# rogosprojects/klogs

Measured on AMD Instinct MI355X. Metric: filtered log GB/s (whole node) at 1/2/4/8 MI355X; % of HBM peak, higher is better.
Workload: dtype u8

## Files before the change

### klogs_amd/csrc/klf_kernels.hip

```cpp
#include <hip/hip_ext.h>
#include <hip/hip_runtime.h>

#include <cstdio>
#include <cstdlib>
#include <cstring>
#include <type_traits>

#include "klf_kernels.hpp"
#include "klf_ts.hpp"

namespace klf {
namespace {

#ifndef KLF_TIMELINE
#define KLF_TIMELINE 0
#endif
__device__ uint32_t g_abl_waves;
#if KLF_TIMELINE
__device__ uint64_t g_timeline[300000 * 8];
__device__ uint32_t g_lb_rounds, g_lb_spins;
#define KLF_STAMP(tile, k) do { if (threadIdx.x == 0 && (tile) < 300000) g_timeline[(size_t)(tile) * 8 + (k)] = __builtin_amdgcn_s_memtime(); } while (0)
#else
#define KLF_STAMP(tile, k) do { } while (0)
#endif
// ... 163 lines not shown
    y.sel = (fl & 2) != 0;
    if (lane >= d) x = f_combine(y, x);
  }
  return x;
}

__device__ __forceinline__ uint32_t xad(uint32_t x, uint32_t c, uint32_t d) {
  uint32_t r;
  asm("v_xad_u32 %0, %1, %2, %3" : "=v"(r) : "v"(x), "s"(c), "v"(d));
  return r;
}
__device__ __forceinline__ uint32_t any_eq16(const uint4& v, uint32_t c4) {
  const uint32_t m = 0xFEFEFEFFu;
  return (xad(v.x, c4, m) | xad(v.y, c4, m) | xad(v.z, c4, m) | xad(v.w, c4, m)) & 0x80808080u;
}
__device__ __forceinline__ uint32_t eq_mask16(const uint4& v, uint32_t c4) {
  auto z = [c4](uint32_t x) {
    const uint32_t y = x ^ c4;
    const uint32_t f = ~(((y & 0x7F7F7F7Fu) + 0x7F7F7F7Fu) | y) & 0x80808080u;
    return (f * 0x00204081u) >> 28;
  };
  return z(v.x) | (z(v.y) << 4) | (z(v.z) << 8) | (z(v.w) << 12);
}

__device__ __forceinline__ uint32_t nor_and(uint32_t a, uint32_t b, uint32_t c) {
  uint32_t r;
  asm("v_bitop3_b32 %0, %1, %2, %3 bitop3:0x02" : "=v"(r) : "v"(a), "v"(b), "s"(c));
  return r;
}
__device__ __forceinline__ uint32_t eq_mask16_nl(const uint4& v) {
  auto z = [](uint32_t x) {
    const uint32_t t = xad(x & 0x7F7F7F7Fu, 0x0A0A0A0Au, 0x7F7F7F7Fu);
    const uint32_t f = nor_and(t, x, 0x80808080u);
    return (f * 0x00204081u) >> 28;
  };
  return z(v.x) | (z(v.y) << 4) | (z(v.z) << 8) | (z(v.w) << 12);
}

template <class T>
__device__ __forceinline__ T wave_max(T x) {
#pragma unroll
  for (int d = 32; d >= 1; d >>= 1) {
    const T o = __shfl_xor(x, d, 64);
    x = o > x ? o : x;
  }
  return x;
}

__device__ __forceinline__ void wave_lds_sync() { asm volatile("s_waitcnt lgkmcnt(0)" ::: "memory"); }

__global__ __launch_bounds__(256) void k_tiles(const SegDesc* segs, uint32_t nsegs, uint32_t ntiles,
                                               uint32_t* tile_seg) {
  for (uint32_t tile = blockIdx.x * 256 + threadIdx.x; tile < ntiles; tile += gridDim.x * 256)
    tile_seg[tile] = find_seg_by_tile(segs, nsegs, tile);
}

__device__ __forceinline__ uint32_t mul_hi_u24(uint32_t a, uint32_t b) {
  uint32_t r;
  asm("v_mul_hi_u32_u24 %0, %1, %2" : "=v"(r) : "s"(b), "v"(a));
  return r;
}
__device__ __forceinline__ uint32_t mul_u24(uint32_t a, uint32_t b) {
  uint32_t r;
  asm("v_mul_u32_u24 %0, %1, %2" : "=v"(r) : "s"(b), "v"(a));
  return r;
}
__device__ __forceinline__ uint32_t mad_u24(uint32_t a, uint32_t b, uint32_t c) {
  uint32_t r;
  asm("v_mad_u32_u24 %0, %1, %2, %3" : "=v"(r) : "v"(a), "s"(b), "v"(c));
  return r;
}
__device__ __forceinline__ uint32_t bfe_u32(uint32_t a, uint32_t off, uint32_t width) {
  uint32_t r;
  asm("v_bfe_u32 %0, %1, %2, %3" : "=v"(r) : "v"(a), "n"(off), "n"(width));
  return r;
}
__device__ __forceinline__ uint32_t shr_byte1(uint32_t w, uint32_t h) {
  uint32_t r;
  asm("v_lshrrev_b32_sdwa %0, %1, %2 dst_sel:DWORD dst_unused:UNUSED_PAD src0_sel:BYTE_1 src1_sel:DWORD"
      : "=v"(r) : "v"(h), "v"(w));
  return r;
}
#ifndef KLF_PARSE_UNALIGNED
#define KLF_PARSE_UNALIGNED 1
#endif
__device__ __forceinline__ bool parse_fast(const uint8_t* lds, uint32_t o, const uint32_t (&cut)[6], bool& since_ok) {
  uint32_t w[8];
  if (KLF_PARSE_UNALIGNED) {
    typedef uint32_t u32x4 __attribute__((ext_vector_type(4)));
    u32x4 x0, x1;
    __builtin_memcpy(&x0, lds + o, 16);
    __builtin_memcpy(&x1, lds + o + 16, 16);
    w[0] = x0.x; w[1] = x0.y; w[2] = x0.z; w[3] = x0.w;
    w[4] = x1.x; w[5] = x1.y; w[6] = x1.z; w[7] = x1.w;
  } else {
    const uint32_t* s32 = reinterpret_cast<const uint32_t*>(lds);
    const uint32_t base = o >> 2, sh = o & 3u;
    uint32_t prev = s32[base];
#pragma unroll
    for (int j = 0; j < 8; ++j) {
      const uint32_t nx = s32[base + j + 1];
      w[j] = __builtin_amdgcn_alignbyte(nx, prev, sh);
      prev = nx;
    }
  }
  const uint32_t sep = ((w[1] ^ 0x2D00002Du) & 0xFF0000FFu) | ((w[2] ^ 0x00540000u) & 0x00FF0000u) |
                       ((w[3] ^ 0x00003A00u) & 0x0000FF00u) | ((w[4] ^ 0x2E00003Au) & 0xFF0000FFu) |
                       ((w[7] ^ 0x00205A00u) & 0x00FFFF00u);
  const uint32_t p0 = __builtin_amdgcn_perm(0u, w[0], 0x00010203u);
  const uint32_t p1 = __builtin_amdgcn_perm(w[2], w[1], 0x01020405u);
  const uint32_t p2 = __builtin_amdgcn_perm(w[3], w[2], 0x03040607u);
  const uint32_t p3 = __builtin_amdgcn_perm(w[5], w[4], 0x01020405u);
  const uint32_t p4 = __builtin_amdgcn_perm(w[6], w[5], 0x02030405u);
  const uint32_t p5 = __builtin_amdgcn_perm(w[7], w[6], 0x02030C04u) | 0x00003000u;
  const uint32_t hi = ((p0 ^ 0x30303030u) | (p1 ^ 0x30303030u) | (p2 ^ 0x30303030u) | (p3 ^ 0x30303030u) |
                       (p4 ^ 0x30303030u) | (p5 ^ 0x30303030u)) & 0xF0F0F0F0u;
  const uint32_t lo = ((p0 + 0x06060606u) | (p1 + 0x06060606u) | (p2 + 0x06060606u) | (p3 + 0x06060606u) |
                       (p4 + 0x06060606u) | (p5 + 0x06060606u)) & 0x40404040u;
  if ((sep | hi | lo) != 0u) return false;
  if (p0 - 0x31393730u > 0x32303939u - 0x31393730u) return false;
  if ((p1 >> 16) - 0x3031u > 0x3132u - 0x3031u) return false;
  if ((p2 >> 16) > 0x3233u || (p2 & 0xFFFFu) > 0x3539u || (p3 >> 16) > 0x3539u) return false;
  if ((p1 & 0xFFFFu) - 0x3031u > 0x3238u - 0x3031u) {
    const uint32_t day = ((p1 >> 8) & 15u) * 10u + (p1 & 15u);
    const uint32_t month = ((p1 >> 24) & 15u) * 10u + ((p1 >> 16) & 15u);
    const uint32_t yy = ((p0 >> 8) & 15u) * 10u + (p0 & 15u);
    const uint32_t dim = month == 2u ? 28u + ((yy & 3u) == 0u ? 1u : 0u) : 30u + ((month + (month >> 3)) & 1u);
    if (day - 1u >= dim) return false;
  }
  const uint64_t a0 = (uint64_t)p0 << 32 | p1, a1 = (uint64_t)p2 << 32 | p3, a2 = (uint64_t)p4 << 32 | p5;
  const uint64_t c0 = (uint64_t)cut[0] << 32 | cut[1], c1 = (uint64_t)cut[2] << 32 | cut[3],
                 c2 = (uint64_t)cut[4] << 32 | cut[5];
  since_ok = a0 > c0 || (a0 == c0 && (a1 > c1 || (a1 == c1 && a2 >= c2)));
  return true;
}

#ifndef KLF_ABL
#define KLF_ABL 0
#endif
#ifndef KLF_SCAN_NT
#define KLF_SCAN_NT 1
#endif
#ifndef KLF_SCAN_PRIO
#define KLF_SCAN_PRIO 0
#endif
#ifndef KLF_NL_MASK
#define KLF_NL_MASK 1
#endif
#ifndef KLF_SCAN_BALLOT
#define KLF_SCAN_BALLOT 1
#endif
#ifndef KLF_SCAN_PACKSUM
#define KLF_SCAN_PACKSUM 1
#endif
#ifndef KLF_VERIFY_PAR
#define KLF_VERIFY_PAR 0
#endif
#ifndef KLF_HIT_INLINE
#define KLF_HIT_INLINE 0
#endif
#ifndef KLF_TS_INLINE
#define KLF_TS_INLINE 1
#endif
#ifndef KLF_SCAN_SUMSKIP
#define KLF_SCAN_SUMSKIP 1
#endif
typedef uint32_t klf_v4u __attribute__((ext_vector_type(4)));
__device__ __forceinline__ uint4 ld_nt(const uint4* p) {
  const klf_v4u v = __builtin_nontemporal_load(reinterpret_cast<const klf_v4u*>(p));
  return make_uint4(v.x, v.y, v.z, v.w);
}
#ifndef KLF_CG_NT
#define KLF_CG_NT 0
#endif
#ifndef KLF_CG_GRID
#define KLF_CG_GRID 8
#endif
#ifndef KLF_CG_PF2
#define KLF_CG_PF2 1
#endif
#ifndef KLF_COPY_U
#define KLF_COPY_U 1
#endif
#ifndef KLF_ANY_BATCH
#define KLF_ANY_BATCH 8
#endif
#ifndef KLF_SCAN_OCC
#define KLF_SCAN_OCC 3
#endif
constexpr int kScanPlain = 0, kScanLit = 1, kScanGen = 2;

__device__ __forceinline__ void copy_tile_runs(const uint8_t* s_buf, uint32_t* s_run, uint16_t* s_map, uint32_t nr,
                                               uint32_t kept, uint64_t obase, uint8_t* out, int lane);

template <int MODE, int QS, int QK, int QQ = 4, bool QA = false, bool FUSE = false>
__global__ __launch_bounds__(kThreads, MODE == kScanGen ? 3 : KLF_SCAN_OCC) void k_scan(RunArgs a, const uint32_t* __restrict__ tseg,
                                                               const SegDesc* __restrict__ segs) {
  static_assert(!FUSE || MODE == kScanPlain, "the fused compaction runs in the plain scan");
  constexpr bool LIT = MODE == kScanLit;
  constexpr bool GEN = MODE == kScanGen;
  constexpr bool ANC = GEN && QA;
  static_assert(QQ == 3 || QQ == 4, "3- or 4-byte grams");
  constexpr int kWaves = kThreads / 64;
  constexpr int kRows = kTile / 1024;
  constexpr int kPad = FUSE ? 16 : 0;
  __shared__ __attribute__((aligned(16))) uint8_t s_tile_all[kWaves][kPad + kTile + kHalo];
  __shared__ __attribute__((aligned(16))) uint32_t s_frun_all[FUSE ? kWaves : 1][FUSE ? kTcRuns : 1];
  __shared__ __attribute__((aligned(16))) uint16_t s_fmap_all[FUSE ? kWaves : 1][FUSE ? kTcChunks : 8];
  __shared__ __attribute__((aligned(16))) uint32_t s_list_all[kWaves][kSlotStride];
  __shared__ __attribute__((aligned(16))) uint32_t s_lit[kMaxFusedLiteral / 4 + 1];
  __shared__ uint4 s_gstat[GEN ? 1 : kWaves][kScanGroup];
  __shared__ uint32_t s_qf[GEN ? kQfWords : 1];
  __shared__ uint32_t s_h2[GEN ? kWaves : 1][1];
  const int t = threadIdx.x, lane = t & 63, wv = __builtin_amdgcn_readfirstlane(t >> 6);
  uint8_t* s_tile = s_tile_all[wv] + kPad;
  uint32_t* s_list = s_list_all[wv];
  uint32_t* err_flag = a.counters + 2;
  for (uint32_t i = t; i < kMaxFusedLiteral / 4 + 1; i += kThreads)
    s_lit[i] = (LIT && i < (a.lit_len + 3) / 4) ? a.lit_words[i] : 0u;
  if (GEN)
    for (uint32_t i = t; i < kQfWords; i += kThreads) s_qf[i] = a.pats.qf_bitmap[i];
  __syncthreads();
  const uint32_t nwaves = gridDim.x * kWaves;
  const bool abl = (KLF_ABL != 0) &&
                   __hip_atomic_load(&g_abl_waves, __ATOMIC_RELAXED, __HIP_MEMORY_SCOPE_AGENT) >= nwaves;
#define ABL(x) ((KLF_ABL & (x)) && abl)

  static_assert(kRows == 8, "KLF_ROWS lists the 8 prefetch rows");
#define KLF_ROWS(X) X(0) X(1) X(2) X(3) X(4) X(5) X(6) X(7)
#define KLF_DECL(r) uint4 pf##r;
  KLF_ROWS(KLF_DECL)
#undef KLF_DECL
#define KLF_LOAD(r) pf##r = (KLF_SCAN_NT && MODE != kScanPlain) ? ld_nt(&gp[r * 64 + lane]) : gp[r * 64 + lane];
#define KLF_STORE(r) l[r * 64 + lane] = pf##r;
  uint4 pfh = make_uint4(0, 0, 0, 0);
  auto next_tile = [&](uint32_t x) -> uint32_t {
    return (FUSE || (x % kScanGroup) != kScanGroup - 1) ? x + 1 : x + 1 + kScanGroup * (nwaves - 1);
  };
  const uint32_t gw = blockIdx.x * kWaves + wv;
  uint32_t tile = FUSE ? gw * a.fuse_range : gw * kScanGroup;
  const uint32_t tile_end = FUSE ? (tile + a.fuse_range < a.ntiles ? tile + a.fuse_range : a.ntiles) : a.ntiles;
  const uint32_t range_t0 = tile;
  uint4 stv = make_uint4(0, 0, 0, 0);
  uint32_t pf_s = 0;
  SegDesc pf_sd{};
  if (tile < a.ntiles) {
    pf_s = tseg[tile];
    pf_sd = segs[pf_s];
    const uint4* gp = reinterpret_cast<const uint4*>(a.bytes + pf_sd.base + (uint64_t)(tile - pf_sd.tile0) * kTile);
    KLF_ROWS(KLF_LOAD)
    if (lane < kHalo / 16) pfh = (KLF_SCAN_NT && MODE != kScanPlain) ? ld_nt(&gp[kTile / 16 + lane]) : gp[kTile / 16 + lane];
  }
  {
    const __amdgpu_buffer_rsrc_t none = __builtin_amdgcn_make_buffer_rsrc(a.slots, 0, 0, 0x00020000);
    __builtin_amdgcn_raw_buffer_store_b32(0u, none, 0x7FFF0000u, 0, 0);
  }
  bool any_defer = false;
  uint32_t wp_cur = 0, wp_end = 0;
  bool fz_known = false, fz_sel = false, fz_res_set = false;
  int32_t fz_crel = -1;
  uint64_t fz_obase = 0, fz_estart = 0, fz_res = 0, fz_part = 0, fz_rbase = 0;
  uint32_t fz_ext = 0;
  if (FUSE && tile < tile_end) {
    fz_rbase = pf_sd.base + (uint64_t)(tile - pf_sd.tile0) * kTile;
    fz_ext = a.fuse_ext0[gw];
  }
  auto fz_close = [&]() __attribute__((always_inline)) {
    if (!fz_res_set) {
      fz_res = fz_part;
      fz_res_set = true;
      fz_estart = fz_obase = fz_rbase + fz_part;
    }
    if (lane == 0) {
      a.fuse_ext[2 * (size_t)fz_ext] = fz_estart;
      a.fuse_ext[2 * (size_t)fz_ext + 1] = fz_obase - fz_estart;
    }
  };
  for (; tile < tile_end; tile = next_tile(tile)) {
    const uint32_t s = pf_s;
    const SegDesc sd = pf_sd;
    const int64_t rel_lo = (int64_t)(tile - sd.tile0) * kTile;
    const int64_t seg_len = (int64_t)sd.len;
    const int32_t tile_len = (int32_t)(seg_len - rel_lo < kTile ? seg_len - rel_lo : kTile);
    const bool first = rel_lo == 0;
    const bool last = rel_lo + kTile >= seg_len;
    const uint8_t* segp = a.bytes + sd.base;

    if (KLF_SCAN_PRIO) __builtin_amdgcn_s_setprio(KLF_SCAN_PRIO);
    {
      uint4* l = reinterpret_cast<uint4*>(s_tile);
      KLF_ROWS(KLF_STORE)
      if (lane < kHalo / 16) l[kTile / 16 + lane] = pfh;
      const uint32_t nx = next_tile(tile);
      if (nx < tile_end) {
        if (nx - sd.tile0 >= sd.ntiles) {
          pf_s = tseg[nx];
          pf_sd = segs[pf_s];
        }
        const uint4* gp = reinterpret_cast<const uint4*>(a.bytes + pf_sd.base + (uint64_t)(nx - pf_sd.tile0) * kTile);
        KLF_ROWS(KLF_LOAD)
        if (lane < kHalo / 16) pfh = (KLF_SCAN_NT && MODE != kScanPlain) ? ld_nt(&gp[kTile / 16 + lane]) : gp[kTile / 16 + lane];
      }
    }
    if (KLF_SCAN_PRIO) __builtin_amdgcn_s_setprio(0);
    wave_lds_sync();

    const uint32_t my0 = (uint32_t)lane * kLaneBytes;
    const int nvalid_s = tile_len - (int)my0;
    const int nvalid = nvalid_s <= 0 ? 0 : (nvalid_s >= kLaneBytes ? kLaneBytes : nvalid_s);
// ... 1020 lines not shown
      e.pad[0] = e.pad[1] = 0;
      s_ent[wv][lane] = e;
      if ((ts.flags & 2u) && base < a.cap_lines && a.scatter_mode != 2 && part == 0) {
        int64_t cs = -1;
        for (uint32_t pt = tile; pt > sd.tile0;) {
          --pt;
          const TileStat pst = a.tstat[pt];
          const int64_t prel = (int64_t)(pt - sd.tile0) * kTile;
          const uint32_t pk0 = prel == 0 ? 0 : 1;
          const uint32_t pn = pst.events + 1 > pk0 ? pst.events + 1 - pk0 : 0;
          if (pn == 0) continue;
          const uint32_t v = slot_at(a, pst, pt, pn - 1);
          const uint32_t mt = v >> 16;
          if ((mt & Meta::kParsed) && !(v & kSlotDefer)) cs = prel + (int64_t)(v & kSlotOff) + (mt >> 2);
          break;
        }
        if (cs >= 0 && rel_lo + (int64_t)ts.carry_off - 1 - (int64_t)kCarryBias >= cs)
          atomicOr(&a.bits[base >> 5], 1u << (base & 31));
      }
      if (last && part == 0) {
        const uint64_t lend = base + ts.events;
        if (lend <= a.cap_lines) a.line_off[lend + s] = sd.len;
        else atomicOr(err_flag, 1u);
      }
    }
    const uint32_t incl = wave_incl_scan_add(n, lane);
    s_pre[wv][lane] = incl;
    const uint32_t gtotal = (uint32_t)__builtin_amdgcn_readlane((int)incl, 63);
    const uint32_t lb = (uint32_t)((uint64_t)gtotal * part / P), total = (uint32_t)((uint64_t)gtotal * (part + 1) / P);
    wave_lds_sync();
    for (uint32_t l0 = lb; l0 < total; l0 += 64 * kScatterBatch) {
      uint32_t sl[kScatterBatch], kk[kScatterBatch], jj[kScatterBatch];
#pragma unroll
      for (int u = 0; u < kScatterBatch; ++u) {
        const uint32_t l = l0 + (uint32_t)(u * 64 + lane);
        sl[u] = 0;
        kk[u] = 0;
        jj[u] = 0;
        if (l < total) {
          uint32_t lo = 0, hi = kScatterGroup - 1;
          while (lo < hi) {
            const uint32_t mid = (lo + hi) >> 1;
            if (s_pre[wv][mid] > l) hi = mid; else lo = mid + 1;
          }
          const uint32_t j = l - (lo ? s_pre[wv][lo - 1] : 0u);
          const uint32_t src = s_ent[wv][lo].src;
          const uint32_t* sp = (src & 0x80000000u) ? a.pool + (src & 0x7FFFFFFFu)
                               : (src & 0x40000000u) ? reinterpret_cast<const uint32_t*>(a.tstat + g * kScatterGroup + lo) + 1
                               : a.slots ? a.slots + (size_t)(g * kScatterGroup + lo) * kRecStride + kRecHead : a.pool;
          sl[u] = sp[j];
          kk[u] = lo;
          jj[u] = j;
        }
      }
#pragma unroll
      for (int u = 0; u < kScatterBatch; ++u) {
        const uint32_t l = l0 + (uint32_t)(u * 64 + lane);
        if (l >= total) continue;
        const ScatterEnt& e = s_ent[wv][kk[u]];
        const uint64_t li = e.base + jj[u];
        if (li >= a.cap_lines) { atomicOr(err_flag, 1u); continue; }
#if KLF_ABL & 16384
        a.line_off[li + e.seg] = e.rel_lo;
        a.meta[li] = (uint16_t)(sl[u] & 0u);
#else
        if (a.scatter_mode != 1) {
          a.line_off[li + e.seg] = e.rel_lo + (sl[u] & kSlotOff);
          a.meta[li] = (uint16_t)(sl[u] >> 16);
        }
        if (sl[u] & kSlotHit) atomicOr(&a.bits[li >> 5], 1u << (li & 31));
#endif
      }
    }
    asm volatile("" ::: "memory");
  }
}
__global__ __launch_bounds__(256) void k_scatter(RunArgs a) {
  __shared__ ScatterLds L;
  scatter_body(a, blockIdx.x, gridDim.x, L);
}

__device__ bool ac_match(const DevPatterns& P, const uint8_t* p, int64_t n) {
  uint32_t st = 0;
  for (int64_t i = 0; i < n; ++i) {
    st = P.ac_next[(size_t)st * P.ac_classes + P.ac_class[p[i]]];
    if (P.ac_accept[st]) return true;
  }
  return false;
}

__device__ bool rx_match(const DevPatterns& P, uint32_t r, const uint8_t* p, int64_t n) {
  const uint32_t fl = P.rx_flags[r];
  if (n == 0) return (fl & 2u) != 0;
  if (fl & 1u) return true;
  const uint64_t first = P.rx_first[r], lastm = P.rx_last[r];
  const uint64_t* B = P.rx_b + (size_t)r * P.rx_classes;
  const uint64_t* F = P.rx_follow + (size_t)r * 64;
  uint64_t d = P.rx_init0[r];
  for (int64_t i = 0; i < n; ++i) {
    const uint64_t c = d & B[P.rx_class[p[i]]];
    if (c & lastm) return true;
    uint64_t nd = first, m = c;
    while (m) {
      const int q = __ffsll((unsigned long long)m) - 1;
      m &= m - 1;
      nd |= F[q];
    }
    d = nd;
  }
  return (d & P.rx_end[r]) != 0;
}

__device__ __forceinline__ uint32_t line_plen(const RunArgs& a, uint16_t meta, const uint8_t* segp,
                                              uint64_t start, uint64_t end) {
  uint32_t plen = meta >> 2;
  if (plen == kPlenEscape) {
    plen = 0;
    for (uint64_t q = start; q < end; ++q)
      if (segp[q] == ' ') { plen = (uint32_t)(q - start) + 1; break; }
  }
  return plen;
}

__device__ __forceinline__ uint32_t gword(const uint8_t* p) {
  const uintptr_t a0 = reinterpret_cast<uintptr_t>(p);
  const uint32_t* w = reinterpret_cast<const uint32_t*>(a0 & ~(uintptr_t)3);
  return __builtin_amdgcn_alignbyte(w[1], w[0], (uint32_t)(a0 & 3));
}

constexpr uint32_t kVerifyQ = 256;
struct VerifyQ {
  uint32_t* n;
  uint64_t (*buf)[2];
};
__device__ __forceinline__ void push_candidate(const RunArgs& a, const VerifyQ& q, uint64_t key, uint64_t x) {
  const uint32_t k = atomicAdd(q.n, 1u);
  if (k < kVerifyQ) {
    q.buf[k][0] = key;
    q.buf[k][1] = x;
    return;
  }
  const uint32_t qi = atomicAdd(&a.counters[kCtrQueue], 1u);
  if (qi < a.cand_cap) {
    a.cand[2 * (size_t)qi] = key;
    a.cand[2 * (size_t)qi + 1] = x;
  } else {
    atomicOr(&a.counters[kCtrQOver], 1u);
  }
}
#ifndef KLF_VERIFY_ENT
#define KLF_VERIFY_ENT 4
#endif
constexpr int kVerifyEnt = KLF_VERIFY_ENT;
__device__ void verify_hit_from(const RunArgs& a, uint32_t tile, uint32_t s, const SegDesc& sd, int32_t p,
                                uint32_t gs, uint32_t e0, uint32_t e1, const VerifyQ& vq) {
  const DevPatterns& P = a.pats;
  const uint8_t* segp = a.bytes + sd.base;
  const int64_t rel_lo = (int64_t)(tile - sd.tile0) * kTile;
  auto entry = [&](const uint4 E) {
    const uint32_t m = E.y & 0xFFFFu, ko = (E.y >> 16) & 0xFFu;
    const uint32_t lm = (E.y & kQfLoose) ? 0x20202020u : 0u;
    auto msk_of = [&](uint32_t k) { return m - k >= 4 ? 0xFFFFFFFFu : ((1u << (8 * (m - k))) - 1u); };
    const int32_t x = p - (int32_t)ko;
    if (rel_lo + x < 0 || rel_lo + x + (int64_t)m > (int64_t)sd.len) return;
    const uint8_t* q = segp + rel_lo + x;
    bool eq = (((gword(q) | lm) ^ P.qf_nbytes[E.x]) & msk_of(0)) == 0;
    if (!KLF_VERIFY_PAR) {
      for (uint32_t k = 4; k < m && eq; k += 4)
        eq = (((gword(q + k) | lm) ^ P.qf_nbytes[E.x + (k >> 2)]) & msk_of(k)) == 0;
    } else if (eq && m > 4) {
      const uintptr_t qa = reinterpret_cast<uintptr_t>(q);
      const uint32_t* qw = reinterpret_cast<const uint32_t*>(qa & ~(uintptr_t)3);
      const uint32_t sh = (uint32_t)(qa & 3);
      uint32_t d[9], want[8];
#pragma unroll
      for (int k = 1; k < 9; ++k) d[k] = (4u * (uint32_t)k < m + 4u) ? qw[k] : 0u;
#pragma unroll
      for (int k = 1; k < 8; ++k) want[k] = 4u * (uint32_t)k < m ? P.qf_nbytes[E.x + (uint32_t)k] : 0u;
#pragma unroll
      for (int k = 1; k < 8; ++k)
        if (4u * (uint32_t)k < m)
          eq = eq && ((((__builtin_amdgcn_alignbyte(d[k + 1], d[k], sh)) | lm) ^ want[k]) & msk_of(4u * (uint32_t)k)) == 0;
      for (uint32_t k = 32; k < m && eq; k += 4)
        eq = (((gword(q + k) | lm) ^ P.qf_nbytes[E.x + (k >> 2)]) & msk_of(k)) == 0;
    }
    if (!eq) return;
#if KLF_ABL & 32
    atomicOr(&a.counters[13], x);
    return;
#endif
    KLF_VSTAMP(2);
    const TileStat ts = a.tstat[tile];
    const bool first = rel_lo == 0, last = rel_lo + kTile >= (int64_t)sd.len;
    const uint32_t k0 = first ? 0 : 1, k1 = last ? ts.events : ts.events + 1;
    const uint32_t nl = k1 > k0 ? k1 - k0 : 0;
    int lo = 0, hi = x < 0 ? 0 : (int)nl;
    while (lo < hi) {
      const int mid = (lo + hi) >> 1;
      if ((int32_t)(slot_at(a, ts, tile, (uint32_t)mid) & kSlotOff) <= x) lo = mid + 1; else hi = mid;
    }
    const uint64_t l = a.tile_base[tile] + (lo > 0 ? k0 + (uint32_t)lo - 1 : 0);
    if (l >= a.cap_lines) {
      atomicOr(&a.counters[2], 1u);
      return;
    }
    KLF_VSTAMP(3);
    uint32_t v = 0;
    int64_t vrel = rel_lo;
    if (lo > 0 || (KLF_ABL & 524288)) {
      v = slot_at(a, ts, tile, lo > 0 ? (uint32_t)lo - 1 : 0u);
    } else {
      for (uint32_t pt = tile; pt > sd.tile0;) {
        --pt;
        const TileStat pst = a.tstat[pt];
        const int64_t prel = (int64_t)(pt - sd.tile0) * kTile;
        const uint32_t pk0 = prel == 0 ? 0u : 1u;
        const uint32_t pn = pst.events + 1 - pk0;
        if (pn == 0) continue;
        v = slot_at(a, pst, pt, pn - 1);
        vrel = prel;
        break;
      }
    }
    const uint16_t mt = (uint16_t)(v >> 16);
    const uint64_t ls = (uint64_t)vrel + (v & kSlotOff);
    KLF_VSTAMP(4);
    if (!(mt & Meta::kParsed)) return;
    if (!(E.y & kQfRegex)) {
      const uint32_t plen = (mt >> 2) == kPlenEscape ? line_plen(a, mt, segp, ls, sd.len) : mt >> 2;
      if ((uint64_t)(rel_lo + x) >= ls + plen) {
        atomicOr(&a.bits[l >> 5], 1u << (l & 31));
        if (a.count_pats) count_pair(a, l, s, E.z);
      }
      return;
    }
    if (!a.count_pats && ((a.bits[l >> 5] >> (l & 31)) & 1u)) return;
    KLF_VSTAMP(5);
    if (a.win_index) {
      uint64_t le = sd.len;
      if ((uint32_t)lo < nl) {
        le = (uint64_t)rel_lo + (slot_at(a, ts, tile, (uint32_t)lo) & kSlotOff);
      } else if (!(KLF_ABL & 262144)) {
        for (uint32_t pt = tile + 1; pt < sd.tile0 + sd.ntiles; ++pt) {
          const TileStat pst = a.tstat[pt];
          const int64_t prel = (int64_t)(pt - sd.tile0) * kTile;
          const uint32_t pk1 = prel + kTile >= (int64_t)sd.len ? pst.events : pst.events + 1;
          if (pk1 <= 1u) continue;
          le = (uint64_t)prel + (slot_at(a, pst, pt, 0) & kSlotOff);
          break;
        }
      }
      a.line_off[l + s] = ls;
      a.line_off[l + s + 1] = le;
      a.meta[l] = mt;
    }
    KLF_VSTAMP(6);
    push_candidate(a, vq, l | ((uint64_t)E.z << 40), (uint64_t)(rel_lo + x) | ((uint64_t)s << 40));
  };
  for (uint32_t eb = e0; eb < e1; eb += kVerifyEnt) {
    uint4 Eb[kVerifyEnt];
    uint32_t pass = 0;
#pragma unroll
    for (int j = 0; j < kVerifyEnt; ++j) Eb[j] = eb + (uint32_t)j < e1 ? P.qf_ent[eb + (uint32_t)j] : make_uint4(0, 0, 0, 0);
#pragma unroll
    for (int j = 0; j < kVerifyEnt; ++j) {
      const uint32_t m = Eb[j].y & 0xFFFFu, ko = (Eb[j].y >> 16) & 0xFFu;
      const uint32_t lm = (Eb[j].y & kQfLoose) ? 0x20202020u : 0u;
      const uint32_t mk = m - ko >= 4 ? 0xFFFFFFFFu : ((1u << (8 * (m - ko))) - 1u);
      if (eb + (uint32_t)j < e1 && (((gs | lm) ^ Eb[j].w) & mk) == 0u) pass |= 1u << j;
    }
    while (pass) {
      const int j = __builtin_ctz(pass);
      pass &= pass - 1u;
      uint4 E = Eb[0];
#pragma unroll
      for (int i = 1; i < kVerifyEnt; ++i)
        if (j == i) E = Eb[i];
      entry(E);
    }
  }
}

__device__ void verify_hit(const RunArgs& a, uint32_t tile, uint32_t s, int32_t p, const VerifyQ& vq) {
  const DevPatterns& P = a.pats;
  const SegDesc sd = a.segs[s];
  const int64_t rel_lo = (int64_t)(tile - sd.tile0) * kTile;
  const uint32_t gs = gword(a.bytes + sd.base + rel_lo + p);
  const uint32_t g = (gs | P.qf_fold) & P.qf_mask;
  const uint32_t b = qf_bucket(g, P.qf_w24, P.qf_k);
  verify_hit_from(a, tile, s, sd, p, gs, P.qf_head[b], P.qf_head[b + 1], vq);
}

constexpr int kVerifyBatch = 4;
struct VerifyLds {
  uint32_t qn[4];
  uint64_t qbuf[4][kVerifyQ][2];
};
__device__ __forceinline__ void verify_body(RunArgs& a, uint32_t bid, uint32_t nb, VerifyLds& L) {
  auto& s_qn = L.qn;
  auto& s_qbuf = L.qbuf;
  if (a.counters[2] || a.counters[kCtrHitsOver]) return;
  const int lane = threadIdx.x & 63, wv = threadIdx.x >> 6;
  if (lane == 0) s_qn[wv] = 0;
  wave_lds_sync();
  const VerifyQ vq{&s_qn[wv], s_qbuf[wv]};
  const uint32_t gid = bid * blockDim.x + threadIdx.x, stride = nb * blockDim.x;
  const uint32_t nf = a.counters[kCtrFlatHits];
  const DevPatterns& P = a.pats;
  if (gid < nf) KLF_VSTAMP(0);
  for (uint32_t i0 = gid; i0 < nf; i0 += kVerifyBatch * stride) {
    uint32_t tile[kVerifyBatch], sg[kVerifyBatch], e0[kVerifyBatch], e1[kVerifyBatch];
    int32_t pp[kVerifyBatch];
    SegDesc sd[kVerifyBatch];
#pragma unroll
    for (int u = 0; u < kVerifyBatch; ++u) {
      const uint32_t i = i0 + (uint32_t)u * stride;
      const uint64_t hf = a.hflat[i < nf ? i : i0];
      tile[u] = (uint32_t)hf;
      pp[u] = (int32_t)((hf >> 32) & 0xFFFFu);
      sg[u] = (uint32_t)(hf >> 48);
      if (sg[u] == 0xFFFFu) sg[u] = a.tile_seg[tile[u]];
    }
#pragma unroll
    for (int u = 0; u < kVerifyBatch; ++u) sd[u] = a.segs[sg[u]];
    uint32_t gg[kVerifyBatch];
#pragma unroll
    for (int u = 0; u < kVerifyBatch; ++u) {
      const int64_t rel_lo = (int64_t)(tile[u] - sd[u].tile0) * kTile;
      gg[u] = gword(a.bytes + sd[u].base + rel_lo + pp[u]);
    }
#pragma unroll
    for (int u = 0; u < kVerifyBatch; ++u) {
      const uint32_t b = qf_bucket((gg[u] | P.qf_fold) & P.qf_mask, P.qf_w24, P.qf_k);
      e0[u] = P.qf_head[b];
      e1[u] = P.qf_head[b + 1];
    }
    KLF_VSTAMP(1);
#pragma unroll
    for (int u = 0; u < kVerifyBatch; ++u)
      if (i0 + (uint32_t)u * stride < nf) {
#if KLF_ABL & 16
        if (pp[u] == 0x7FFF) atomicOr(&a.counters[13], sg[u]);
        continue;
#endif
        verify_hit_from(a, tile[u], sg[u], sd[u], pp[u], gg[u], e0[u], e1[u], vq);
      }
  }
  const uint32_t nh = a.counters[kCtrHits] < a.qhits_cap ? a.counters[kCtrHits] : a.qhits_cap;
  for (uint32_t i = gid; i < nh; i += stride) {
    const uint64_t pos = a.qhits[i];
    uint32_t lo = 0, hi = a.nsegs;
    while (hi - lo > 1) {
      const uint32_t mid = (lo + hi) >> 1;
      if (a.segs[mid].base <= pos) lo = mid; else hi = mid;
    }
    const uint64_t rel = pos - a.segs[lo].base;
    const uint32_t tile = a.segs[lo].tile0 + (uint32_t)(rel / kTile);
    verify_hit(a, tile, lo, (int32_t)(rel % kTile), vq);
  }
  if (gid == 0) a.counters[kCtrVerified] = nf + nh;
  if (gid < nf) KLF_VSTAMP(7);
  wave_lds_sync();
  const uint32_t nq = s_qn[wv] < kVerifyQ ? s_qn[wv] : kVerifyQ;
  if (nq) {
    uint32_t base = 0;
    if (lane == 0) base = atomicAdd(&a.counters[kCtrQueue], nq);
    base = (uint32_t)__builtin_amdgcn_readfirstlane((int)base);
    for (uint32_t k = (uint32_t)lane; k < nq; k += 64) {
      if ((uint64_t)base + k < a.cand_cap) {
        a.cand[2 * ((size_t)base + k)] = s_qbuf[wv][k][0];
        a.cand[2 * ((size_t)base + k) + 1] = s_qbuf[wv][k][1];
      } else {
        atomicOr(&a.counters[kCtrQOver], 1u);
      }
    }
  }
}
#ifndef KLF_VERIFY_WAVES
#define KLF_VERIFY_WAVES 4
#endif
__global__ __launch_bounds__(256, KLF_VERIFY_WAVES) void k_verify(RunArgs a) {
  __shared__ VerifyLds L;
  verify_body(a, blockIdx.x, gridDim.x, L);
}
__global__ __launch_bounds__(256, KLF_VERIFY_WAVES) void k_scatter_verify(RunArgs a, uint32_t nsb) {
  __shared__ union {
    ScatterLds s;
    VerifyLds v;
  } L;
  if (blockIdx.x < nsb) scatter_body(a, blockIdx.x, nsb, L.s);
  else verify_body(a, blockIdx.x - nsb, gridDim.x - nsb, L.v);
}

struct NfaTables {
  const uint8_t* cls;
  const uint64_t* b;
  const uint64_t* fol;
  const uint64_t* vec;
  uint32_t classes, fstride;
};

__device__ __forceinline__ uint64_t nfa_chunk(const NfaTables& T, uint32_t r, const uint8_t* p, uint64_t n,
                                              uint64_t d, bool inject, bool& hit) {
  const uint64_t* V = T.vec + 4 * (size_t)r;
  const uint64_t first = inject ? V[0] : 0ull, lastm = V[1];
  const uint64_t* B = T.b + (size_t)r * T.classes;
  const uint64_t* F = T.fol + (size_t)r * T.fstride;
  const uintptr_t a0 = reinterpret_cast<uintptr_t>(p);
  const uint4* q = reinterpret_cast<const uint4*>(a0 & ~(uintptr_t)15);
  uint32_t skip = (uint32_t)(a0 & 15);
  uint64_t left = n;
  while (left) {
    if (!inject && d == 0) return 0;
    const uint4 v = *q++;
    const uint32_t w[4] = {v.x, v.y, v.z, v.w};
    uint64_t bm[16];
#pragma unroll
    for (int j = 0; j < 16; ++j) bm[j] = B[T.cls[(w[j >> 2] >> (8 * (j & 3))) & 0xFFu]];
    const uint32_t j0 = skip;
    const uint32_t j1 = (uint64_t)(16 - skip) < left ? 16u : skip + (uint32_t)left;
    left -= j1 - j0;
    skip = 0;
#pragma unroll
    for (uint32_t j = 0; j < 16; ++j) {
      if (j < j0 || j >= j1) continue;
      const uint64_t c = d & bm[j];
      if (c & lastm) { hit = true; return 0; }
      uint64_t nd = first;
      for (uint64_t m = c; m; m &= m - 1) nd |= F[__ffsll((unsigned long long)m) - 1];
      d = nd;
    }
  }
  return d;
}

__device__ bool nfa_wave(const NfaTables& T, uint32_t r, const uint8_t* p, uint64_t n, int lane) {
  const uint64_t* V = T.vec + 4 * (size_t)r;
  const uint64_t first = V[0];
  uint64_t L = (n + 63) / 64;
  L = (L + 15) & ~15ull;
  const uint32_t nc = (uint32_t)((n + L - 1) / L);
  const bool mine = (uint32_t)lane < nc;
  const uint64_t lo = mine ? (uint64_t)lane * L : 0, hi = mine ? (lo + L < n ? lo + L : n) : 0;
  bool hit = false;
  uint64_t e = 0;
  if (mine) e = nfa_chunk(T, r, p + lo, hi - lo, lane == 0 ? V[2] : first, true, hit);
  if (__any(hit)) return true;
  uint64_t fin = (uint32_t)lane == nc - 1 ? e : 0;
  uint64_t x = __shfl_up(e & ~first, 1, 64);
  if (lane == 0 || !mine) x = 0;
  for (int round = 0; round < 64 && __any(x != 0); ++round) {
    uint64_t y = 0;
    if (x) y = nfa_chunk(T, r, p + lo, hi - lo, x, false, hit);
    if (__any(hit)) return true;
    if ((uint32_t)lane == nc - 1) fin |= y;
    x = __shfl_up(y, 1, 64);
    if (lane == 0 || !mine) x = 0;
  }
  const uint64_t f = __shfl(fin, (int)nc - 1, 64);
  return (f & V[3]) != 0;
}

template <bool LDS>
__global__ __launch_bounds__(256) void k_nfa(RunArgs a) {
  extern __shared__ uint64_t s_nfa[];
  if (a.counters[2] || a.counters[kCtrQOver] || a.counters[kCtrHitsOver]) return;
  const uint32_t nq = a.counters[kCtrQueue] < a.cand_cap ? a.counters[kCtrQueue] : a.cand_cap;
  if (nq == 0 || blockIdx.x * (blockDim.x / 64) >= nq) return;
  const DevPatterns& P = a.pats;
  const uint32_t R = P.rx_count, C = P.rx_classes, FS = LDS ? P.rx_maxpos : 64;
  NfaTables T;
  if (LDS) {
    uint64_t* sb = s_nfa;
    uint64_t* sf = sb + (size_t)R * C;
    uint64_t* sv = sf + (size_t)R * FS;
    uint8_t* sc = reinterpret_cast<uint8_t*>(sv + 4 * (size_t)R);
    for (uint32_t i = threadIdx.x; i < R * C; i += blockDim.x) sb[i] = P.rx_b[i];
    for (uint32_t i = threadIdx.x; i < R * FS; i += blockDim.x) sf[i] = P.rx_follow[(size_t)(i / FS) * 64 + i % FS];
    for (uint32_t i = threadIdx.x; i < R; i += blockDim.x) {
      sv[4 * i] = P.rx_first[i];
      sv[4 * i + 1] = P.rx_last[i];
      sv[4 * i + 2] = P.rx_init0[i];
      sv[4 * i + 3] = P.rx_end[i];
    }
    for (uint32_t i = threadIdx.x; i < 256; i += blockDim.x) sc[i] = P.rx_class[i];
    __syncthreads();
    T = NfaTables{sc, sb, sf, sv, C, FS};
  } else {
    T = NfaTables{P.rx_class, P.rx_b, P.rx_follow, P.rx_vec, C, 64};
  }
  const int lane = threadIdx.x & 63;
  const uint32_t nw = gridDim.x * (blockDim.x / 64);
  for (uint32_t i = blockIdx.x * (blockDim.x / 64) + (threadIdx.x >> 6); i < nq; i += nw) {
    const uint64_t e = a.cand[2 * (size_t)i];
    const uint64_t l = e & ((1ull << 40) - 1);
    const uint32_t r = (uint32_t)(e >> 40);
    if (P.rx_pre[r] != kRxPreNone) continue;
    const uint32_t s = (uint32_t)(a.cand[2 * (size_t)i + 1] >> 40);
    if (!a.count_pats && ((a.bits[l >> 5] >> (l & 31)) & 1u)) continue;
    const uint16_t m = a.meta[l];
    if (!(m & Meta::kParsed)) continue;
    const uint8_t* segp = a.bytes + a.segs[s].base;
    const uint64_t ls = a.line_off[l + s], le = a.line_off[l + s + 1];
    const uint32_t plen = line_plen(a, m, segp, ls, le);
    uint64_t cs = ls + plen, ce = le;
    if (ce > cs && segp[ce - 1] == '\n') --ce;
    if (ce <= cs) continue;
    const bool hit = (P.rx_flags[r] & 1u) || nfa_wave(T, r, segp + cs, ce - cs, lane);
    if (hit && lane == 0) {
      atomicOr(&a.bits[l >> 5], 1u << (l & 31));
      if (a.count_pats) count_pair(a, l, s, P.n_lits + r);
    }
  }
}

__global__ __launch_bounds__(256) void k_fixcount(RunArgs a) {
  if (!a.counters[kCtrDefer] || a.counters[2]) return;
  if (a.win_index) {
    if (blockIdx.x == 0 && threadIdx.x == 0) a.counters[kCtrRedo] = 1u;
    return;
  }
  const int lane = threadIdx.x & 63, wv = threadIdx.x >> 6;
  for (uint32_t tile = blockIdx.x * 4 + wv; tile < a.ntiles; tile += gridDim.x * 4) {
    const TileStat ts = a.tstat[tile];
    if (!(ts.flags & 4u)) continue;
    const uint32_t s = a.tile_seg[tile];
    const SegDesc sd = a.segs[s];
// ... 2217 lines not shown
```

Baseline: 5554.

## Stage verify candidate pairs in LDS and drain them lane-parallel per wave

```diff
diff --git a/klogs_amd/csrc/klf_kernels.hip b/klogs_amd/csrc/klf_kernels.hip
--- a/klogs_amd/csrc/klf_kernels.hip
+++ b/klogs_amd/csrc/klf_kernels.hip
@@ -339,9 +339,6 @@
 #endif
 #ifndef KLF_SCAN_PACKSUM
 #define KLF_SCAN_PACKSUM 1
-#endif
-#ifndef KLF_VERIFY_PAR
-#define KLF_VERIFY_PAR 0
 #endif
 #ifndef KLF_HIT_INLINE
 #define KLF_HIT_INLINE 0
@@ -1668,45 +1665,61 @@
 #define KLF_VERIFY_ENT 4
 #endif
 constexpr int kVerifyEnt = KLF_VERIFY_ENT;
-__device__ void verify_hit_from(const RunArgs& a, uint32_t tile, uint32_t s, const SegDesc& sd, int32_t p,
-                                uint32_t gs, uint32_t e0, uint32_t e1, const VerifyQ& vq) {
+constexpr uint32_t kVerifyPairs = 128;
+struct VerifyPair {
+  uint32_t ex, ey, ez;
+  uint32_t tile, s;
+  int32_t p;
+  uint64_t q;
+};
+struct VerifyStage {
+  uint32_t* n;
+  VerifyPair* buf;
+};
+#ifndef KLF_VERIFY_NPAR
+#define KLF_VERIFY_NPAR 4
+#endif
+__device__ __forceinline__ void verify_pair(const RunArgs& a, const uint32_t tile, const uint32_t s, const SegDesc& sd,
+                                            const int32_t p, const uint32_t ex, const uint32_t ey, const uint32_t ez,
+                                            const uint8_t* q, const VerifyQ& vq) {
   const DevPatterns& P = a.pats;
   const uint8_t* segp = a.bytes + sd.base;
-  const int64_t rel_lo = (int64_t)(tile - sd.tile0) * kTile;
-  auto entry = [&](const uint4 E) {
+  {
+    struct { uint32_t x, y, z; } E{ex, ey, ez};
     const uint32_t m = E.y & 0xFFFFu, ko = (E.y >> 16) & 0xFFu;
     const uint32_t lm = (E.y & kQfLoose) ? 0x20202020u : 0u;
     auto msk_of = [&](uint32_t k) { return m - k >= 4 ? 0xFFFFFFFFu : ((1u << (8 * (m - k))) - 1u); };
     const int32_t x = p - (int32_t)ko;
-    if (rel_lo + x < 0 || rel_lo + x + (int64_t)m > (int64_t)sd.len) return;
-    const uint8_t* q = segp + rel_lo + x;
-    bool eq = (((gword(q) | lm) ^ P.qf_nbytes[E.x]) & msk_of(0)) == 0;
-    if (!KLF_VERIFY_PAR) {
-      for (uint32_t k = 4; k < m && eq; k += 4)
-        eq = (((gword(q + k) | lm) ^ P.qf_nbytes[E.x + (k >> 2)]) & msk_of(k)) == 0;
-    } else if (eq && m > 4) {
+    bool eq;
+    constexpr int NP = KLF_VERIFY_NPAR;
+    uint32_t d[NP + 1], want[NP];
+    {
       const uintptr_t qa = reinterpret_cast<uintptr_t>(q);
       const uint32_t* qw = reinterpret_cast<const uint32_t*>(qa & ~(uintptr_t)3);
-      const uint32_t sh = (uint32_t)(qa & 3);
-      uint32_t d[9], want[8];
-#pragma unroll
-      for (int k = 1; k < 9; ++k) d[k] = (4u * (uint32_t)k < m + 4u) ? qw[k] : 0u;
-#pragma unroll
-      for (int k = 1; k < 8; ++k) want[k] = 4u * (uint32_t)k < m ? P.qf_nbytes[E.x + (uint32_t)k] : 0u;
-#pragma unroll
-      for (int k = 1; k < 8; ++k)
+#pragma unroll
+      for (int k = 0; k <= NP; ++k) d[k] = (4u * (uint32_t)k < m + 4u) ? qw[k] : 0u;
+#pragma unroll
+      for (int k = 0; k < NP; ++k) want[k] = 4u * (uint32_t)k < m ? P.qf_nbytes[E.x + (uint32_t)k] : 0u;
+    }
+    const TileStat ts = a.tstat[tile];
+    const uint64_t tbase = a.tile_base[tile];
+    {
+      const uint32_t sh = (uint32_t)(reinterpret_cast<uintptr_t>(q) & 3);
+      eq = true;
+#pragma unroll
+      for (int k = 0; k < NP; ++k)
         if (4u * (uint32_t)k < m)
           eq = eq && ((((__builtin_amdgcn_alignbyte(d[k + 1], d[k], sh)) | lm) ^ want[k]) & msk_of(4u * (uint32_t)k)) == 0;
-      for (uint32_t k = 32; k < m && eq; k += 4)
-        eq = (((gword(q + k) | lm) ^ P.qf_nbytes[E.x + (k >> 2)]) & msk_of(k)) == 0;
-    }
+    }
+    const int64_t rel_lo = (int64_t)(tile - sd.tile0) * kTile;
+    for (uint32_t k = 4u * NP; k < m && eq; k += 4)
+      eq = (((gword(q + k) | lm) ^ P.qf_nbytes[E.x + (k >> 2)]) & msk_of(k)) == 0;
     if (!eq) return;
 #if KLF_ABL & 32
     atomicOr(&a.counters[13], x);
     return;
 #endif
     KLF_VSTAMP(2);
-    const TileStat ts = a.tstat[tile];
     const bool first = rel_lo == 0, last = rel_lo + kTile >= (int64_t)sd.len;
     const uint32_t k0 = first ? 0 : 1, k1 = last ? ts.events : ts.events + 1;
     const uint32_t nl = k1 > k0 ? k1 - k0 : 0;
@@ -1715,7 +1728,7 @@
       const int mid = (lo + hi) >> 1;
       if ((int32_t)(slot_at(a, ts, tile, (uint32_t)mid) & kSlotOff) <= x) lo = mid + 1; else hi = mid;
     }
-    const uint64_t l = a.tile_base[tile] + (lo > 0 ? k0 + (uint32_t)lo - 1 : 0);
+    const uint64_t l = tbase + (lo > 0 ? k0 + (uint32_t)lo - 1 : 0);
     if (l >= a.cap_lines) {
       atomicOr(&a.counters[2], 1u);
       return;
@@ -1772,7 +1785,14 @@
     }
     KLF_VSTAMP(6);
     push_candidate(a, vq, l | ((uint64_t)E.z << 40), (uint64_t)(rel_lo + x) | ((uint64_t)s << 40));
-  };
+  }
+}
+
+__device__ __forceinline__ void verify_walk(const RunArgs& a, uint32_t tile, uint32_t s, int32_t p, uint32_t gs,
+                                            uint32_t e0, uint32_t e1, const VerifyStage& st, const VerifyQ& vq) {
+  const DevPatterns& P = a.pats;
+  const SegDesc sd = a.segs[s];
+  const int64_t rel_lo = (int64_t)(tile - sd.tile0) * kTile;
   for (uint32_t eb = e0; eb < e1; eb += kVerifyEnt) {
     uint4 Eb[kVerifyEnt];
     uint32_t pass = 0;
@@ -1792,46 +1812,86 @@
 #pragma unroll
       for (int i = 1; i < kVerifyEnt; ++i)
         if (j == i) E = Eb[i];
-      entry(E);
-    }
-  }
-}
-
-__device__ void verify_hit(const RunArgs& a, uint32_t tile, uint32_t s, int32_t p, const VerifyQ& vq) {
+      const uint32_t m = E.y & 0xFFFFu, ko = (E.y >> 16) & 0xFFu;
+      const int64_t rx = rel_lo + ((int64_t)p - (int64_t)ko);
+      if (rx < 0 || rx + (int64_t)m > (int64_t)sd.len) continue;
+      const uint64_t q = sd.base + (uint64_t)rx;
+      const uint32_t k = atomicAdd(st.n, 1u);
+      if (k < kVerifyPairs) {
+        st.buf[k] = VerifyPair{E.x, E.y, E.z, tile, s, p, q};
+      } else {
+        verify_pair(a, tile, s, sd, p, E.x, E.y, E.z, a.bytes + q, vq);
+      }
+    }
+  }
+}
+__device__ __forceinline__ void verify_drain(const RunArgs& a, const VerifyStage& st, const VerifyQ& vq, int lane, bool all) {
+  wave_lds_sync();
+  uint32_t n = (uint32_t)__builtin_amdgcn_readfirstlane((int)*st.n);
+  if (n == 0 || (!all && n < 64u)) return;
+  n = n < kVerifyPairs ? n : kVerifyPairs;
+  for (uint32_t k = (uint32_t)lane; k < n; k += 64) {
+    const VerifyPair pr = st.buf[k];
+    const SegDesc sd = a.segs[pr.s];
+    verify_pair(a, pr.tile, pr.s, sd, pr.p, pr.ex, pr.ey, pr.ez, a.bytes + pr.q, vq);
+  }
+  wave_lds_sync();
+  if (lane == 0) *st.n = 0;
+  wave_lds_sync();
+}
+
+__device__ __forceinline__ void verify_hit(const RunArgs& a, uint32_t tile, uint32_t s, int32_t p, const VerifyStage& st,
+                                           const VerifyQ& vq) {
   const DevPatterns& P = a.pats;
   const SegDesc sd = a.segs[s];
   const int64_t rel_lo = (int64_t)(tile - sd.tile0) * kTile;
   const uint32_t gs = gword(a.bytes + sd.base + rel_lo + p);
   const uint32_t g = (gs | P.qf_fold) & P.qf_mask;
   const uint32_t b = qf_bucket(g, P.qf_w24, P.qf_k);
-  verify_hit_from(a, tile, s, sd, p, gs, P.qf_head[b], P.qf_head[b + 1], vq);
+  verify_walk(a, tile, s, p, gs, P.qf_head[b], P.qf_head[b + 1], st, vq);
 }
 
 constexpr int kVerifyBatch = 4;
+#ifndef KLF_VERIFY_HPW
+#define KLF_VERIFY_HPW 32
+#endif
+constexpr uint32_t kVerifyHpw = KLF_VERIFY_HPW;
 struct VerifyLds {
   uint32_t qn[4];
+  uint32_t pn[4];
+  uint32_t done;
   uint64_t qbuf[4][kVerifyQ][2];
+  VerifyPair pbuf[4][kVerifyPairs];
 };
+static_assert(sizeof(VerifyLds) <= 40 * 1024, "four verify blocks share a CU's LDS");
 __device__ __forceinline__ void verify_body(RunArgs& a, uint32_t bid, uint32_t nb, VerifyLds& L) {
   auto& s_qn = L.qn;
   auto& s_qbuf = L.qbuf;
-  if (a.counters[2] || a.counters[kCtrHitsOver]) return;
   const int lane = threadIdx.x & 63, wv = threadIdx.x >> 6;
-  if (lane == 0) s_qn[wv] = 0;
-  wave_lds_sync();
+  if (lane == 0) { s_qn[wv] = 0; L.pn[wv] = 0; }
+  if (threadIdx.x == 0) L.done = 0;
+  __syncthreads();
+  const bool skip = a.counters[2] || a.counters[kCtrHitsOver];
   const VerifyQ vq{&s_qn[wv], s_qbuf[wv]};
-  const uint32_t gid = bid * blockDim.x + threadIdx.x, stride = nb * blockDim.x;
-  const uint32_t nf = a.counters[kCtrFlatHits];
+  const VerifyStage st{&L.pn[wv], L.pbuf[wv]};
+  const uint32_t nw = nb * (blockDim.x >> 6), wid = bid * (blockDim.x >> 6) + (uint32_t)wv;
+  const uint32_t nf = skip ? 0u : a.counters[kCtrFlatHits];
+  const uint64_t hpw_fill = ((uint64_t)nf + nw / 2 - 1) / (nw / 2);
+  const uint32_t hpw = hpw_fill < kVerifyHpw ? kVerifyHpw : hpw_fill > 64 ? 64u : (uint32_t)hpw_fill;
+  const uint64_t round = (uint64_t)nw * hpw;
   const DevPatterns& P = a.pats;
-  if (gid < nf) KLF_VSTAMP(0);
-  for (uint32_t i0 = gid; i0 < nf; i0 += kVerifyBatch * stride) {
+  const bool work = (uint64_t)wid * hpw < nf;
+  if (work) KLF_VSTAMP(0);
+  for (uint64_t b0 = (uint64_t)wid * hpw; b0 < nf; b0 += kVerifyBatch * round) {
     uint32_t tile[kVerifyBatch], sg[kVerifyBatch], e0[kVerifyBatch], e1[kVerifyBatch];
     int32_t pp[kVerifyBatch];
     SegDesc sd[kVerifyBatch];
+    bool act[kVerifyBatch];
 #pragma unroll
     for (int u = 0; u < kVerifyBatch; ++u) {
-      const uint32_t i = i0 + (uint32_t)u * stride;
-      const uint64_t hf = a.hflat[i < nf ? i : i0];
+      const uint64_t i = b0 + (uint64_t)u * round + (uint32_t)lane;
+      act[u] = (uint32_t)lane < hpw && i < nf;
+      const uint64_t hf = a.hflat[act[u] ? i : b0];
       tile[u] = (uint32_t)hf;
       pp[u] = (int32_t)((hf >> 32) & 0xFFFFu);
       sg[u] = (uint32_t)(hf >> 48);
@@ -1852,43 +1912,75 @@
       e1[u] = P.qf_head[b + 1];
     }
     KLF_VSTAMP(1);
-#pragma unroll
-    for (int u = 0; u < kVerifyBatch; ++u)
-      if (i0 + (uint32_t)u * stride < nf) {
+#pragma nounroll
+    for (int u = 0; u < kVerifyBatch; ++u) {
+      uint32_t tile_u = tile[0], sg_u = sg[0], e0_u = e0[0], e1_u = e1[0], gg_u = gg[0];
+      int32_t pp_u = pp[0];
+      bool act_u = act[0];
+#pragma unroll
+      for (int i = 1; i < kVerifyBatch; ++i)
+        if (u == i) {
+          tile_u = tile[i]; sg_u = sg[i]; e0_u = e0[i]; e1_u = e1[i]; gg_u = gg[i];
+          pp_u = pp[i]; act_u = act[i];
+        }
+      if (act_u) {
 #if KLF_ABL & 16
-        if (pp[u] == 0x7FFF) atomicOr(&a.counters[13], sg[u]);
+        if (pp_u == 0x7FFF) atomicOr(&a.counters[13], sg_u);
         continue;
 #endif
-        verify_hit_from(a, tile[u], sg[u], sd[u], pp[u], gg[u], e0[u], e1[u], vq);
-      }
-  }
-  const uint32_t nh = a.counters[kCtrHits] < a.qhits_cap ? a.counters[kCtrHits] : a.qhits_cap;
-  for (uint32_t i = gid; i < nh; i += stride) {
-    const uint64_t pos = a.qhits[i];
-    uint32_t lo = 0, hi = a.nsegs;
-    while (hi - lo > 1) {
-      const uint32_t mid = (lo + hi) >> 1;
-      if (a.segs[mid].base <= pos) lo = mid; else hi = mid;
-    }
-    const uint64_t rel = pos - a.segs[lo].base;
-    const uint32_t tile = a.segs[lo].tile0 + (uint32_t)(rel / kTile);
-    verify_hit(a, tile, lo, (int32_t)(rel % kTile), vq);
-  }
-  if (gid == 0) a.counters[kCtrVerified] = nf + nh;
-  if (gid < nf) KLF_VSTAMP(7);
+        verify_walk(a, tile_u, sg_u, pp_u, gg_u, e0_u, e1_u, st, vq);
+      }
+      verify_drain(a, st, vq, lane, u == kVerifyBatch - 1);
+    }
+  }
+  const uint32_t nh = skip ? 0u : a.counters[kCtrHits] < a.qhits_cap ? a.counters[kCtrHits] : a.qhits_cap;
+  for (uint64_t b0 = (uint64_t)wid * 64; b0 < nh; b0 += (uint64_t)nw * 64) {
+    const uint64_t i = b0 + (uint32_t)lane;
+    if (i < nh) {
+      const uint64_t pos = a.qhits[i];
+      uint32_t lo = 0, hi = a.nsegs;
+      while (hi - lo > 1) {
+        const uint32_t mid = (lo + hi) >> 1;
+        if (a.segs[mid].base <= pos) lo = mid; else hi = mid;
+      }
+      const uint64_t rel = pos - a.segs[lo].base;
+      const uint32_t tile = a.segs[lo].tile0 + (uint32_t)(rel / kTile);
+      verify_hit(a, tile, lo, (int32_t)(rel % kTile), st, vq);
+    }
+    verify_drain(a, st, vq, lane, true);
+  }
+  if (wid == 0 && lane == 0 && !skip) a.counters[kCtrVerified] = nf + nh;
+  if (work) KLF_VSTAMP(7);
   wave_lds_sync();
-  const uint32_t nq = s_qn[wv] < kVerifyQ ? s_qn[wv] : kVerifyQ;
+  uint32_t arrived = 0;
+  if (lane == 0) arrived = atomicAdd(&L.done, 1u);
+  if ((uint32_t)__builtin_amdgcn_readfirstlane((int)arrived) + 1u != (blockDim.x >> 6)) return;
+  wave_lds_sync();
+  uint32_t nqw[4], nq = 0;
+#pragma unroll
+  for (int w = 0; w < 4; ++w) {
+    nqw[w] = (uint32_t)w < (blockDim.x >> 6) ? (s_qn[w] < kVerifyQ ? s_qn[w] : kVerifyQ) : 0u;
+    nq += nqw[w];
+  }
   if (nq) {
     uint32_t base = 0;
+#if KLF_ABL & 1048576
+    base = bid * 4 * kVerifyQ;
+#else
     if (lane == 0) base = atomicAdd(&a.counters[kCtrQueue], nq);
+#endif
     base = (uint32_t)__builtin_amdgcn_readfirstlane((int)base);
-    for (uint32_t k = (uint32_t)lane; k < nq; k += 64) {
-      if ((uint64_t)base + k < a.cand_cap) {
-        a.cand[2 * ((size_t)base + k)] = s_qbuf[wv][k][0];
-        a.cand[2 * ((size_t)base + k) + 1] = s_qbuf[wv][k][1];
-      } else {
-        atomicOr(&a.counters[kCtrQOver], 1u);
-      }
+#pragma unroll
+    for (int w = 0; w < 4; ++w) {
+      for (uint32_t k = (uint32_t)lane; k < nqw[w]; k += 64) {
+        if ((uint64_t)base + k < a.cand_cap) {
+          a.cand[2 * ((size_t)base + k)] = s_qbuf[w][k][0];
+          a.cand[2 * ((size_t)base + k) + 1] = s_qbuf[w][k][1];
+        } else {
+          atomicOr(&a.counters[kCtrQOver], 1u);
+        }
+      }
+      base += nqw[w];
     }
   }
 }
```

Result: no change. 5606 (median of 6 runs) (+0.9%).
